# XJay18/NeuMA

Measured on AMD Instinct MI355X. Metric: sim+render frames/sec (fwd+bwd), 100k pts / 128^3 grid / 1080p, higher is better.
Workload: dtype f32; 1 GPU; metric: 100000 particles / 128^3 grid / 200000 Gaussians / 1920x1080; substeps_per_frame=20, views_per_frame=3, sh_degree=3, material=jelly_0300 + LoRA r16, parallelism=single GPU, start_state=rest

## Files before the change

### neuma_amd/csrc/nm_material.hip

```cpp
#include "nm_common.h"
#include "nm_grid.h"
#include <cstddef>

typedef float f4 __attribute__((ext_vector_type(4)));
#ifdef NM_PHASES
__device__ long long g_nm_phase[3 * 8 * 2048];
extern "C" int nm_debug_phases(long long* out, int n) {
  return hipMemcpyFromSymbol(out, HIP_SYMBOL(g_nm_phase), (size_t)n * sizeof(long long)) == hipSuccess ? 0 : -2;
}
#define NM_PH_DECL long long ph_t0 = clock64(); long long ph[8] = {0, 0, 0, 0, 0, 0, 0, 0};
#define NM_PH(i) { long long t1 = clock64(); ph[i] += t1 - ph_t0; ph_t0 = t1; }
#define NM_PH_STORE_K(kind) if ((threadIdx.x & 63) == 0) { int w = blockIdx.x * 4 + (threadIdx.x >> 6); if (w < 2048) for (int i = 0; i < 8; ++i) g_nm_phase[((kind) * 2048 + w) * 8 + i] = ph[i]; }
#define NM_PH_STORE NM_PH_STORE_K(0)
#else
#define NM_PH_STORE_K(kind)
#define NM_PH_DECL
#define NM_PH(i)
#define NM_PH_STORE
#endif
#define NM_MFMA(a, b, c) __builtin_amdgcn_mfma_f32_16x16x4f32((a), (b), (c), 0, 0, 0)
#define NM_SB_() __builtin_amdgcn_sched_barrier(0)

#define NM_BWD_GRID 256
#define NM_PRO_WGS 32
#define NM_PROLOGUE_SPLIT(pro) material_prologue(pro)
__device__ __forceinline__ bool material_prologue(const GridPrologue& pro) {
  if (pro.mode == 0) return false;
  const int mat = pro.mat_grid;
  if ((int)gridDim.x > mat) {
    if ((int)blockIdx.x < mat) return false;
    grid_prologue(pro, blockIdx.x - mat, gridDim.x - mat);
    return true;
  }
  grid_prologue(pro, blockIdx.x, gridDim.x);
  return false;
}
__device__ __forceinline__ bool material_prologue_fwd(const GridPrologue& pro) {
  if (pro.mode == 0) return false;
  const int mat = pro.mat_grid;
  if ((int)gridDim.x > mat) {
    if ((int)blockIdx.x < mat) return false;
    grid_prologue_clear(pro, blockIdx.x - mat, gridDim.x - mat);
    return true;
  }
  grid_prologue_clear(pro, blockIdx.x, gridDim.x);
  return false;
}
#define NM_W0 (64 * 13)
#define NM_W1 (64 * 64)
#define NM_W2 (9 * 64)
#define NM_WTOT (NM_W0 + NM_W1 + NM_W2)
#define NM_WACC_W0 (64 * 64)
#define NM_WACC_W2 (64 * 64 + 16 * 64)
#define NM_WACC (64 * 64 + 16 * 64 + 16 * 64)
__host__ __device__ inline int wacc_to_plain(int e) {
  const int reg = e & 3, lane = (e >> 2) & 63, blk = e >> 8, g = lane >> 4, j = lane & 15;
  if (blk < 16) return NM_W0 + (16 * (blk >> 2) + 4 * g + reg) * 64 + 16 * (blk & 3) + j;
  if (blk < 20) return j < 13 ? (16 * (blk - 16) + 4 * g + reg) * 13 + j : -1;
  return 4 * g + reg < 9 ? NM_W0 + NM_W1 + (4 * g + reg) * 64 + 16 * (blk - 20) + j : -1;
// ... 170 lines not shown
  __device__ __forceinline__ void operator()() const {}
};
template <int NFLOAT, class HOOK = NoHook>
__device__ __forceinline__ void stage_permuted(const float* __restrict__ wperm, float* dst, HOOK between = HOOK()) {
  constexpr int NV = NFLOAT / 4, PER = (NV + 255) / 256;
  float4 v[PER];
#pragma unroll
  for (int k = 0; k < PER; ++k) {
    int i = threadIdx.x + 256 * k;
    v[k] = i < NV ? reinterpret_cast<const float4*>(wperm)[i] : make_float4(0.f, 0.f, 0.f, 0.f);
  }
  NM_SB_();
  between();
  NM_SB_();
#pragma unroll
  for (int k = 0; k < PER; ++k) {
    int i = threadIdx.x + 256 * k;
    if (i < NV) reinterpret_cast<float4*>(dst)[i] = v[k];
  }
}
template <int NA, int NB, int NHOOK, class HOOK>
__device__ __forceinline__ void stage_permuted2(const float* __restrict__ srca, float* dsta, const float* __restrict__ srcb, float* dstb,
                                                HOOK between) {
  constexpr int VA = NA / 4, PA = (VA + 255) / 256, VB = NB / 4, PB = (VB + 255) / 256;
  f4 va[PA], vb[PB];
#pragma unroll
  for (int k = 0; k < PA; ++k) {
    const int i = threadIdx.x + 256 * k;
    const f4* ptr = reinterpret_cast<const f4*>(srca) + (i < VA ? i : VA - 1);
    asm volatile("global_load_dwordx4 %0, %1, off" : "=v"(va[k]) : "v"(ptr));
  }
#pragma unroll
  for (int k = 0; k < PB; ++k) {
    const int i = threadIdx.x + 256 * k;
    const f4* ptr = reinterpret_cast<const f4*>(srcb) + (i < VB ? i : VB - 1);
    asm volatile("global_load_dwordx4 %0, %1, off" : "=v"(vb[k]) : "v"(ptr));
  }
  asm volatile("" ::: "memory");
  between();
  static_assert(NHOOK >= 0 && NHOOK < 48, "vmcnt is a 6-bit counter");
  asm volatile("s_waitcnt vmcnt(%0)" ::"n"(NHOOK) : "memory");
#pragma unroll
  for (int k = 0; k < PA; ++k) {
    const int i = threadIdx.x + 256 * k;
    asm volatile("" : "+v"(va[k]));
    if (i < VA) *reinterpret_cast<f4*>(dsta + 4 * i) = va[k];
  }
#pragma unroll
  for (int k = 0; k < PB; ++k) {
    const int i = threadIdx.x + 256 * k;
    asm volatile("" : "+v"(vb[k]));
    if (i < VB) *reinterpret_cast<f4*>(dstb + 4 * i) = vb[k];
  }
}
__global__ void __launch_bounds__(256) k_permute_weights(const float* __restrict__ w0, const float* __restrict__ w1,
                                                         const float* __restrict__ w2, float* __restrict__ wperm,
                                                         const float* __restrict__ w0b, const float* __restrict__ w1b,
                                                         const float* __restrict__ w2b, float* __restrict__ wpermb) {
  __shared__ float raw[NM_RAWTOT];
  if (blockIdx.x == 1) { w0 = w0b; w1 = w1b; w2 = w2b; wperm = wpermb; }
  __shared__ float perm[NM_PERM_ALL];
  stage_raw_weights(w0, w1, w2, raw);
  __syncthreads();
  stage_fwd_weights(raw, perm, perm + 16 * 64, perm + 16 * 64 + 64 * 64);
  stage_bwd_weights(raw, perm + NM_PERM_FWD, perm + NM_PERM_FWD + 16 * 64, perm + NM_PERM_FWD + 16 * 64 + 64 * 64);
  __syncthreads();
  for (int i = threadIdx.x; i < NM_PERM_ALL; i += 256) wperm[i] = perm[i];
}

__device__ __forceinline__ void svd_store(float* __restrict__ dst, int n, int p, const M3& U, const float s[3], const M3& V) {
#pragma unroll
  for (int c = 0; c < 9; ++c) __builtin_nontemporal_store(U.m[c], &dst[(size_t)c * n + p]);
#pragma unroll
  for (int c = 0; c < 3; ++c) __builtin_nontemporal_store(s[c], &dst[(size_t)(9 + c) * n + p]);
#pragma unroll
  for (int c = 0; c < 9; ++c) __builtin_nontemporal_store(V.m[c], &dst[(size_t)(12 + c) * n + p]);
}
__device__ __forceinline__ void svd_load(const float* __restrict__ src, int n, int p, M3& U, float s[3], M3& V) {
#pragma unroll
  for (int c = 0; c < 9; ++c) U.m[c] = __builtin_nontemporal_load(&src[(size_t)c * n + p]);
#pragma unroll
  for (int c = 0; c < 3; ++c) s[c] = __builtin_nontemporal_load(&src[(size_t)(9 + c) * n + p]);
#pragma unroll
  for (int c = 0; c < 9; ++c) V.m[c] = __builtin_nontemporal_load(&src[(size_t)(12 + c) * n + p]);
}
template <bool HAVE_SVD = false>
__device__ __forceinline__ void nm_features(const M3& F, float z[13], M3& R, M3& U, M3& V, float s[3]) {
  if (!HAVE_SVD) nm_svd3(F, U, s, V);
  R = m3_mul_nt(U, V);
  M3 G = m3_mul_tn(F, F);
  z[0] = s[0] - 1.f; z[1] = s[1] - 1.f; z[2] = s[2] - 1.f;
#pragma unroll
  for (int i = 0; i < 9; ++i) z[3 + i] = G.m[i] - ((i % 4 == 0) ? 1.f : 0.f);
  z[12] = m3_det(F) - 1.f;
}

#define NM_SB() __builtin_amdgcn_sched_barrier(0)
template <int G>
struct AGroup {
  float a[G];
};
template <int G>
__device__ __forceinline__ void a_fetch(AGroup<G>& o, const float* __restrict__ base, int lane, int grp) {
  static_assert(G % 4 == 0, "groups of four operands (one 16-byte read each)");
#pragma unroll
  for (int q = 0; q < G / 4; ++q) {
// ... 303 lines not shown
    NM_LAUNCH(k_material_fwd_pair<true>, dim3(launch), dim3(256), 0, s, n, q, alpha_p, wperm_p, wperm_e, F_next, stress_next, gp, *g2p,
              svd_p, svd_e, ap, ae);
  else
    NM_LAUNCH(k_material_fwd_pair<false>, dim3(launch), dim3(256), 0, s, n, q, alpha_p, wperm_p, wperm_e, F_next, stress_next, gp, *g2p,
              svd_p, svd_e, ap, ae);
  NM_LAUNCH_CHECK();
  return NM_OK;
}
int nm_material_prepare(const nm_mlp* w, float* wperm, void* stream) {
  NM_LAUNCH(k_permute_weights, dim3(1), dim3(256), 0, (hipStream_t)stream, w->w0, w->w1, w->w2, wperm, (const float*)nullptr,
            (const float*)nullptr, (const float*)nullptr, (float*)nullptr);
  NM_LAUNCH_CHECK();
  return NM_OK;
}
int nm_material_prepare2(const nm_mlp* wa, float* wperm_a, const nm_mlp* wb, float* wperm_b, void* stream) {
  NM_LAUNCH(k_permute_weights, dim3(2), dim3(256), 0, (hipStream_t)stream, wa->w0, wa->w1, wa->w2, wperm_a, wb->w0, wb->w1, wb->w2,
            wperm_b);
  NM_LAUNCH_CHECK();
  return NM_OK;
}
size_t nm_material_prepared_floats() { return NM_PERM_ALL; }

extern "C" int nm_material_fwd(int32_t n, int32_t kind, float alpha, const float* F, const nm_mlp* w, float* out,
                               void* stream) {
  NM_REQUIRE(n >= 0, "negative n");
  NM_REQUIRE(kind == NM_ELASTICITY || kind == NM_PLASTICITY, "kind must be NM_ELASTICITY or NM_PLASTICITY");
  if (n == 0) return NM_OK;
  NM_REQUIRE(F && out && w && w->w0 && w->w1 && w->w2, "null pointer");
  return nm_material_fwd_launch(n, kind, alpha, F, w, nullptr, out, nullptr, nullptr, stream);
}

struct BwdFuse {
  const float* trial_C;
  const int* enabled;
  float dt;
  int add_to_gF;
  int polar;
  const float* svd_in;
};
struct BwdWave {
  float Z[64 * 17];
  float GY[64 * 13];
  float Y[64 * 9];
  float GZ[64 * 13];
  float TA[64 * 17];
  float TB[64 * 17];
  float TC[64 * 17];
};
struct BwdLds {
  float P0[16 * 64], P1[64 * 64], P2[16 * 64];
  float Q0[16 * 64], Q1[64 * 64], Q2[12 * 64];
  BwdWave W[4];
};

struct BwdArgs {
  int n, q;
  float alpha;
  const float *F, *w0, *w1, *w2, *wperm, *gout;
  float *gF, *wpart;
  int want_w;
  BwdFuse fz;
  const f4* act;
};

template <int KIND, bool ACT, bool WW = false>
__device__ __forceinline__ void material_bwd_body(const BwdArgs& a, char* smem_raw) {
  const int n = a.n, q = a.q, wmode = a.want_w;
  const bool want_w = WW ? true : (wmode != 0);
  const float alpha = a.alpha;
  const float* __restrict__ F = a.F;
  const float *__restrict__ w0 = a.w0, *__restrict__ w1 = a.w1, *__restrict__ w2 = a.w2, *__restrict__ wperm = a.wperm;
  const float* __restrict__ gout = a.gout;
  float *__restrict__ gF = a.gF, *__restrict__ wpart = a.wpart;
  const BwdFuse fz = a.fz;
  BwdLds& L = *reinterpret_cast<BwdLds*>(smem_raw);
  NM_PH_DECL
  const int wave = threadIdx.x >> 6, lane = threadIdx.x & 63;
  const int pbeg = min(n, (blockIdx.x * 4 + wave) * q), pend = min(n, pbeg + q);
  struct M3Raw {
    f4 a, b;
    float c;
  };
  typedef float f4u __attribute__((ext_vector_type(4), aligned(4)));
  auto raw_load = [](const float* __restrict__ ptr, M3Raw& r) {
    r.a = *reinterpret_cast<const f4u*>(ptr); r.b = *reinterpret_cast<const f4u*>(ptr + 4); r.c = ptr[8];
  };
  auto raw_m3 = [](const M3Raw& r) {
    M3 m;
    m.m[0] = r.a[0]; m.m[1] = r.a[1]; m.m[2] = r.a[2]; m.m[3] = r.a[3];
    m.m[4] = r.b[0]; m.m[5] = r.b[1]; m.m[6] = r.b[2]; m.m[7] = r.b[3]; m.m[8] = r.c;
    return m;
  };
  struct RoundIn {
    int en_p;
    M3Raw Fp, go, T;
    M3 U, V;
    float s[3];
  };
  f4 nx[ACT ? NM_ACT_SLOTS : 1];
  auto load_first_act = [&](int c0_) {
    if (ACT) {
      const f4* at_ = a.act + (size_t)(c0_ >> 4) * NM_ACT_SLOTS * 64 + lane;
#pragma unroll
      for (int k = 0; k < NM_ACT_SLOTS; ++k) nx[k] = __builtin_nontemporal_load(&at_[k * 64]);
    }
  };
  auto load_round = [&](int c0_, RoundIn& o) {
    const int p_ = c0_ + lane;
    const bool valid_ = p_ < pend;
    o.en_p = (fz.trial_C && valid_) ? fz.enabled[p_] : 0;
    if (valid_) {
      raw_load(F + (size_t)9 * p_, o.Fp);
      raw_load(gout + (size_t)9 * p_, o.go);
      if (fz.trial_C) raw_load(fz.trial_C + (size_t)9 * p_, o.T);
    }
    if (fz.svd_in) {
      if (valid_) svd_load(fz.svd_in, n, p_, o.U, o.s, o.V);
      else { o.U = m3_ident(); o.V = m3_ident(); o.s[0] = o.s[1] = o.s[2] = 1.f; }
    }
  };
  RoundIn ahead;
  if (pbeg < pend) load_round(pbeg, ahead);
  NM_SB();
  if (wperm) {
    static_assert(offsetof(BwdLds, W) == NM_PERM_ALL * sizeof(float), "P0..Q2 must be contiguous in operand order");
    if (ACT) {
      stage_permuted2<16 * 64, NM_PERM_ALL - NM_PERM_FWD, NM_ACT_SLOTS>(wperm, L.P0, wperm + NM_PERM_FWD, L.Q0,
                                                          [&]() { load_first_act(pbeg < pend ? pbeg : 0); });
    } else {
      stage_permuted<NM_PERM_ALL>(wperm, L.P0);
    }
    __syncthreads();
  } else {
    static_assert(sizeof(BwdWave) * 4 >= NM_RAWTOT * sizeof(float), "raw weights must fit the per-wave buffers");
    float* raw = &L.W[0].Z[0];
    stage_raw_weights(w0, w1, w2, raw);
    __syncthreads();
    stage_fwd_weights(raw, L.P0, L.P1, L.P2);
    stage_bwd_weights(raw, L.Q0, L.Q1, L.Q2);
    __syncthreads();
  }
  NM_PH(0)
  const int j = lane & 15, g = lane >> 4;
  float* zb = L.W[wave].Z;
  float* gyb = L.W[wave].GY;
  float* yb = L.W[wave].Y;
  float* gzb = L.W[wave].GZ;
  float* ta = L.W[wave].TA;
  float* tb = L.W[wave].TB;
  float* tc = L.W[wave].TC;
  const f4 zero = {0.f, 0.f, 0.f, 0.f};
  f4 gW1[4][4], gW0[4], gW2[4];
#pragma unroll
  for (int a = 0; a < 4; ++a) {
    gW0[a] = zero; gW2[a] = zero;
#pragma unroll
    for (int b = 0; b < 4; ++b) gW1[a][b] = zero;
  }
  for (int c0 = pbeg; c0 < pend; c0 += 64) {
    const int p = c0 + lane;
    const bool valid = p < pend;
    const int ntile = (min(64, pend - c0) + 15) >> 4;
    const f4* act_tile = ACT ? a.act + (size_t)(c0 >> 4) * NM_ACT_SLOTS * 64 + lane : nullptr;
    M3 Fp = valid ? raw_m3(ahead.Fp) : m3_ident(), go = valid ? raw_m3(ahead.go) : m3_zero();
    M3 T = (fz.trial_C && valid) ? raw_m3(ahead.T) : m3_zero();
    M3 R, U = ahead.U, V = ahead.V;
    float z[13], s[3] = {ahead.s[0], ahead.s[1], ahead.s[2]};
    const bool trial = ahead.en_p != 0;
    if (c0 + 64 < pend) load_round(c0 + 64, ahead);
    NM_SB();
    if (fz.trial_C && !trial) { Fp = m3_ident(); T = m3_zero(); }
    if (trial) {
#pragma unroll
      for (int i = 0; i < 9; ++i) T.m[i] *= fz.dt;
      T.m[0] += 1.f; T.m[4] += 1.f; T.m[8] += 1.f;
      Fp = m3_mul(T, Fp);
    }
    if (fz.svd_in) nm_features<true>(Fp, z, R, U, V, s);
    else nm_features(Fp, z, R, U, V, s);
#pragma unroll
    for (int c = 0; c < 13; ++c) zb[lane * 17 + c] = z[c];
    zb[lane * 17 + 13] = 0.f; zb[lane * 17 + 14] = 0.f; zb[lane * 17 + 15] = 0.f;
    M3 Rtg = m3_mul_tn(R, go);
    M3 Xb;
    if (KIND == NM_ELASTICITY) Xb = m3_mul(Rtg, Fp);
    else {
#pragma unroll
      for (int i = 0; i < 9; ++i) Xb.m[i] = alpha * Rtg.m[i];
    }
#pragma unroll
    for (int r = 0; r < 3; ++r)
#pragma unroll
      for (int c = 0; c < 3; ++c) gyb[lane * 13 + 3 * r + c] = 0.5f * (Xb.m[3 * r + c] + Xb.m[3 * c + r]);
    gyb[lane * 13 + 9] = 0.f; gyb[lane * 13 + 10] = 0.f; gyb[lane * 13 + 11] = 0.f; gyb[lane * 13 + 12] = 0.f;
    __builtin_amdgcn_wave_barrier();
    NM_PH(1)

#pragma unroll 1
    for (int ct = 0; ct < ntile; ++ct) {
      MlpFwd m;
      if (ACT) {
        f4 h2[4];
#pragma unroll
        for (int rt = 0; rt < 4; ++rt) { h2[rt] = nx[rt]; m.g2[rt] = nx[4 + rt]; }
        m.y = nx[8];
        const bool more = c0 + 16 * (ct + 1) < pend;
        if (more) {
#pragma unroll
          for (int k = 0; k < 5; ++k) nx[k] = __builtin_nontemporal_load(&act_tile[((size_t)(ct + 1) * NM_ACT_SLOTS + k) * 64]);
        }
        float zin[4];
#pragma unroll
        for (int ks = 0; ks < 4; ++ks) zin[ks] = zb[(ct * 16 + j) * 17 + 4 * ks + g];
        AGroup<8> first;
        a_fetch<8>(first, L.P0, lane, 0);
        const f4 zero4 = {0.f, 0.f, 0.f, 0.f};
        f4 a1[4] = {zero4, zero4, zero4, zero4};
        a_chain<16, 8, 3, 2>(first, L.P0, lane, zin, a1, [&]() {
          if (want_w) {
#pragma unroll
            for (int rt = 0; rt < 4; ++rt)
#pragma unroll
              for (int r = 0; r < 4; ++r) tb[(16 * rt + 4 * g + r) * 17 + j] = h2[rt][r];
            __builtin_amdgcn_wave_barrier();
          }
        });
#pragma unroll
        for (int rt = 0; rt < 4; ++rt)
#pragma unroll
          for (int pr = 0; pr < 2; ++pr) {
            f2 h, dh;
            nm_gelu_both2((f2){a1[rt][2 * pr], a1[rt][2 * pr + 1]}, h, dh);
            m.g1[rt][2 * pr] = dh[0];
            m.g1[rt][2 * pr + 1] = dh[1];
            if (want_w) {
              tc[(16 * rt + 4 * g + 2 * pr) * 17 + j] = h[0];
              tc[(16 * rt + 4 * g + 2 * pr + 1) * 17 + j] = h[1];
            }
          }
        __builtin_amdgcn_wave_barrier();
      } else {
        float zin[4];
#pragma unroll
        for (int ks = 0; ks < 4; ++ks) zin[ks] = zb[(ct * 16 + j) * 17 + 4 * ks + g];
        AGroup<8> first;
        a_fetch<8>(first, L.P0, lane, 0);
        mlp_forward_tile<true>(L.P0, L.P1, L.P2, zin, lane, first, m, want_w ? tc : nullptr, want_w ? tb : nullptr);
      }
#pragma unroll
      for (int r = 0; r < 4; ++r) {
        int row = 4 * g + r;
        if (row < 9) yb[(ct * 16 + j) * 9 + row] = m.y[r];
      }
      NM_PH(2)
      const float* gyt = gyb + ct * 16 * 13;
      f4 d2[4] = {zero, zero, zero, zero};
      float w2a[2], w2b[2][4];
      {
        AGroup<4> q2g;
        a_fetch<4>(q2g, L.Q2, lane, 0);
        float b[3];
#pragma unroll
        for (int ks = 0; ks < 3; ++ks) b[ks] = gyt[j * 13 + 4 * ks + g];
        if (want_w) {
          w2a[0] = j < 9 ? gyt[g * 13 + j] : 0.f;
#pragma unroll
          for (int ctp = 0; ctp < 4; ++ctp) w2b[0][ctp] = tb[(16 * ctp + j) * 17 + g];
        }
        a_chain<12, 4, 3, 2>(q2g, L.Q2, lane, b, d2);
      }
#pragma unroll
      for (int rt = 0; rt < 4; ++rt) d2[rt] *= m.g2[rt];
      NM_PH(4)
      AGroup<8> q1g;
      a_fetch<8>(q1g, L.Q1, lane, 0);
      NM_SB();
      if (want_w) {
#pragma unroll
        for (int rt = 0; rt < 4; ++rt)
#pragma unroll
          for (int r = 0; r < 4; ++r) ta[(16 * rt + 4 * g + r) * 17 + j] = d2[rt][r];
        __builtin_amdgcn_wave_barrier();
#pragma unroll
        for (int ks = 0; ks < 4; ++ks) {
          const int c = ks & 1, nx = c ^ 1;
          if (ks < 3) {
            w2a[nx] = j < 9 ? gyt[(4 * (ks + 1) + g) * 13 + j] : 0.f;
#pragma unroll
            for (int ctp = 0; ctp < 4; ++ctp) w2b[nx][ctp] = tb[(16 * ctp + j) * 17 + 4 * (ks + 1) + g];
          }
          NM_SB();
#pragma unroll
          for (int ctp = 0; ctp < 4; ++ctp) gW2[ctp] = NM_MFMA(w2a[c], w2b[c][ctp], gW2[ctp]);
          NM_SB();
        }
      }
      NM_PH(3)
      if (ACT && c0 + 16 * (ct + 1) < pend) {
#pragma unroll
        for (int k = 5; k < NM_ACT_SLOTS; ++k) nx[k] = __builtin_nontemporal_load(&act_tile[((size_t)(ct + 1) * NM_ACT_SLOTS + k) * 64]);
      }
      f4 d1[4] = {zero, zero, zero, zero};
      float w1a[2][4], w1b[2][4];
      {
        float b[16];
#pragma unroll
        for (int rtp = 0; rtp < 4; ++rtp)
#pragma unroll
          for (int reg = 0; reg < 4; ++reg) b[4 * rtp + reg] = d2[rtp][reg];
        if (want_w) {
#pragma unroll
          for (int t = 0; t < 4; ++t) {
            w1b[0][t] = tc[(16 * t + j) * 17 + g];
            w1a[0][t] = ta[(16 * t + j) * 17 + g];
          }
        }
        a_chain<64, 8, 3, 2>(q1g, L.Q1, lane, b, d1);
      }
#pragma unroll
      for (int rt = 0; rt < 4; ++rt) d1[rt] *= m.g1[rt];
      NM_PH(6)
      AGroup<8> q0g;
      a_fetch<8>(q0g, L.Q0, lane, 0);
      NM_SB();
      if (want_w) {
#pragma unroll
        for (int rt = 0; rt < 4; ++rt)
#pragma unroll
          for (int r = 0; r < 4; ++r) tb[(16 * rt + 4 * g + r) * 17 + j] = d1[rt][r];
        __builtin_amdgcn_wave_barrier();
#pragma unroll
        for (int ks = 0; ks < 4; ++ks) {
          const int c = ks & 1, nx = c ^ 1;
          if (ks < 3) {
#pragma unroll
            for (int t = 0; t < 4; ++t) {
              w1b[nx][t] = tc[(16 * t + j) * 17 + 4 * (ks + 1) + g];
              w1a[nx][t] = ta[(16 * t + j) * 17 + 4 * (ks + 1) + g];
            }
          }
          NM_SB();
#pragma unroll
          for (int rt = 0; rt < 4; ++rt)
#pragma unroll
            for (int ctp = 0; ctp < 4; ++ctp) gW1[rt][ctp] = NM_MFMA(w1a[c][rt], w1b[c][ctp], gW1[rt][ctp]);
          NM_SB();
        }
      }
      NM_PH(5)
      f4 dzz[2] = {zero, zero};
      float w0b[2], w0a[2][4];
      {
        float b[16];
#pragma unroll
        for (int rtp = 0; rtp < 4; ++rtp)
#pragma unroll
          for (int reg = 0; reg < 4; ++reg) b[4 * rtp + reg] = d1[rtp][reg];
        if (want_w) {
          w0b[0] = zb[(ct * 16 + g) * 17 + j];
#pragma unroll
          for (int rt = 0; rt < 4; ++rt) w0a[0][rt] = tb[(16 * rt + j) * 17 + g];
        }
        a_chain<16, 8, 1, 0>(q0g, L.Q0, lane, b, dzz);
      }
      const f4 dza = dzz[0] + dzz[1];
#pragma unroll
      for (int r = 0; r < 4; ++r) {
        int row = 4 * g + r;
        if (row < 13) gzb[(ct * 16 + j) * 13 + row] = dza[r];
      }
      if (want_w) {
#pragma unroll
        for (int ks = 0; ks < 4; ++ks) {
          const int c = ks & 1, nx = c ^ 1;
          if (ks < 3) {
            w0b[nx] = zb[(ct * 16 + 4 * (ks + 1) + g) * 17 + j];
#pragma unroll
            for (int rt = 0; rt < 4; ++rt) w0a[nx][rt] = tb[(16 * rt + j) * 17 + 4 * (ks + 1) + g];
          }
          NM_SB();
#pragma unroll
          for (int rt = 0; rt < 4; ++rt) gW0[rt] = NM_MFMA(w0a[c][rt], w0b[c], gW0[rt]);
          NM_SB();
        }
      }
    }
    __builtin_amdgcn_wave_barrier();

    M3Raw prev_raw;
    const bool add_prev = fz.add_to_gF && valid;
    if (add_prev) raw_load(gF + (size_t)9 * p, prev_raw);
    M3 X;
#pragma unroll
    for (int i = 0; i < 9; ++i) X.m[i] = yb[lane * 9 + i];
    M3 Xs;
#pragma unroll
    for (int r = 0; r < 3; ++r)
#pragma unroll
      for (int c = 0; c < 3; ++c) Xs.m[3 * r + c] = 0.5f * (X.m[3 * r + c] + X.m[3 * c + r]);
    float zbv[13];
#pragma unroll
    for (int c = 0; c < 13; ++c) zbv[c] = gzb[lane * 13 + c];
    M3 Fb, Rb;
    if (KIND == NM_ELASTICITY) {
      M3 gFm = m3_mul(go, Fp);
      Rb = m3_mul(gFm, Xs);
      M3 RX = m3_mul(R, Xs);
      Fb = m3_mul_tn(go, RX);
    } else {
      M3 gX = m3_mul(go, Xs);
#pragma unroll
      for (int i = 0; i < 9; ++i) { Rb.m[i] = alpha * gX.m[i]; Fb.m[i] = go.m[i]; }
    }
    M3 At = m3_mul(m3_mul_tn(U, Rb), V);
    M3 inner;
#pragma unroll
    for (int r = 0; r < 3; ++r)
#pragma unroll
      for (int c = 0; c < 3; ++c) {
        if (r == c) { inner.m[4 * r] = zbv[r]; continue; }
        float kf;
        if (fz.polar) {
          float den = s[r] + s[c];
          den = fabsf(den) < 1e-6f ? copysignf(1e-6f, den) : den;
          kf = 1.f / den;
        } else {
          const int a = r < c ? r : c, b = r < c ? c : r;
          kf = (s[b] - s[a]) / fminf(s[b] * s[b] - s[a] * s[a], -1e-6f);
        }
        inner.m[3 * r + c] = (At.m[3 * r + c] - At.m[3 * c + r]) * kf;
      }
    M3 t = m3_mul_nt(m3_mul(U, inner), V);
    M3 Gs;
#pragma unroll
    for (int r = 0; r < 3; ++r)
#pragma unroll
      for (int c = 0; c < 3; ++c) Gs.m[3 * r + c] = zbv[3 + 3 * r + c] + zbv[3 + 3 * c + r];
    M3 FG = m3_mul(Fp, Gs);
    M3 cof = m3_cofactor(Fp);
#pragma unroll
    for (int i = 0; i < 9; ++i) Fb.m[i] += t.m[i] + FG.m[i] + zbv[12] * cof.m[i];
    if (valid) {
      if (add_prev) {
        const M3 prev = raw_m3(prev_raw);
#pragma unroll
        for (int i = 0; i < 9; ++i) Fb.m[i] += prev.m[i];
      }
      m3_store(gF + 9 * p, Fb);
    }
    __builtin_amdgcn_wave_barrier();
    NM_PH(7)
  }
  NM_PH_STORE_K(KIND == NM_PLASTICITY ? 1 : 0)

  if (!want_w) return;
  constexpr int W4 = NM_WACC / 4, WPER = W4 / 256;
  static_assert(W4 % 256 == 0, "whole 16-byte pieces per thread");
  f4* dst = reinterpret_cast<f4*>(wpart + (size_t)blockIdx.x * NM_WACC);
  f4 prev[WPER];
  if (wmode == 2) {
#pragma unroll
    for (int k = 0; k < WPER; ++k) prev[k] = dst[threadIdx.x + 256 * k];
  } else {
#pragma unroll
    for (int k = 0; k < WPER; ++k) prev[k] = zero;
  }
  NM_SB();
  __syncthreads();
  static_assert(sizeof(BwdLds) >= 4 * NM_WACC * sizeof(float), "four weight-gradient copies must fit");
  f4* red = reinterpret_cast<f4*>(smem_raw) + wave * W4;
#pragma unroll
  for (int rt = 0; rt < 4; ++rt) {
#pragma unroll
    for (int ctp = 0; ctp < 4; ++ctp) red[(rt * 4 + ctp) * 64 + lane] = gW1[rt][ctp];
    red[NM_WACC_W0 / 4 + rt * 64 + lane] = gW0[rt];
    red[NM_WACC_W2 / 4 + rt * 64 + lane] = gW2[rt];
  }
  __syncthreads();
  const f4* all = reinterpret_cast<const f4*>(smem_raw);
#pragma unroll
  for (int k = 0; k < WPER; ++k) {
    const int i = threadIdx.x + 256 * k;
    const f4 v = (all[i] + all[W4 + i]) + (all[2 * W4 + i] + all[3 * W4 + i]);
    dst[i] = prev[k] + v;
  }
}

template <int KIND, bool ACT>
__global__ void __launch_bounds__(256, 1) k_material_bwd(BwdArgs a, GridPrologue pro) {
  extern __shared__ __attribute__((aligned(16))) char smem_raw[];
  if (NM_PROLOGUE_SPLIT(pro)) return;
  material_bwd_body<KIND, ACT>(a, smem_raw);
}

template <bool ACT, bool WW>
__global__ void __launch_bounds__(256, 1) k_material_bwd_pair(BwdArgs e, BwdArgs p, GridPrologue pro) {
  extern __shared__ __attribute__((aligned(16))) char smem_raw[];
  if (NM_PROLOGUE_SPLIT(pro)) return;
  material_bwd_body<NM_ELASTICITY, ACT, WW>(e, smem_raw);
  __threadfence_block();
  __syncthreads();
  material_bwd_body<NM_PLASTICITY, ACT, WW>(p, smem_raw);
}

__global__ void __launch_bounds__(256) k_wgrad_reduce(const float* __restrict__ wpart, int nparts, float* __restrict__ g0,
                                                      float* __restrict__ g1, float* __restrict__ g2, int accumulate,
                                                      const float* __restrict__ wpart_b, float* __restrict__ gb) {
  __shared__ float part[4][64];
  if (blockIdx.y == 1) {
    wpart = wpart_b; g0 = gb; g1 = gb + NM_W0; g2 = gb + NM_W0 + NM_W1;
  }
  const int li = threadIdx.x & 63, sl = threadIdx.x >> 6;
  const int e = blockIdx.x * 64 + li;
  const int i = wacc_to_plain(e);
  float acc = 0.f;
  if (i >= 0) {
    float a0 = 0.f, a1 = 0.f, a2 = 0.f, a3 = 0.f;
    int b = sl;
    for (; b + 12 < nparts; b += 16) {
      a0 += wpart[(size_t)b * NM_WACC + e];
      a1 += wpart[(size_t)(b + 4) * NM_WACC + e];
      a2 += wpart[(size_t)(b + 8) * NM_WACC + e];
      a3 += wpart[(size_t)(b + 12) * NM_WACC + e];
    }
    for (; b < nparts; b += 4) a0 += wpart[(size_t)b * NM_WACC + e];
    acc = (a0 + a1) + (a2 + a3);
  }
  part[sl][li] = acc;
  __syncthreads();
  if (sl == 0 && i >= 0) {
    acc = (part[0][li] + part[1][li]) + (part[2][li] + part[3][li]);
    float* dst = i < NM_W0 ? g0 + i : (i < NM_W0 + NM_W1 ? g1 + (i - NM_W0) : g2 + (i - NM_W0 - NM_W1));
    *dst = accumulate ? *dst + acc : acc;
  }
}

static int bwd_attr_once() {
  static bool attr_done[64] = {};
  int devid = 0;
  NM_HIP_CHECK(hipGetDevice(&devid));
  const bool attr_set = devid >= 0 && devid < 64 && attr_done[devid];
  if (!attr_set) {
    NM_HIP_CHECK(hipFuncSetAttribute((const void*)k_material_bwd<NM_ELASTICITY, true>, hipFuncAttributeMaxDynamicSharedMemorySize,
                                     (int)sizeof(BwdLds)));
    NM_HIP_CHECK(hipFuncSetAttribute((const void*)k_material_bwd<NM_PLASTICITY, true>, hipFuncAttributeMaxDynamicSharedMemorySize,
                                     (int)sizeof(BwdLds)));
    NM_HIP_CHECK(hipFuncSetAttribute((const void*)k_material_bwd_pair<true, true>, hipFuncAttributeMaxDynamicSharedMemorySize,
                                     (int)sizeof(BwdLds)));
    NM_HIP_CHECK(hipFuncSetAttribute((const void*)k_material_bwd_pair<true, false>, hipFuncAttributeMaxDynamicSharedMemorySize,
                                     (int)sizeof(BwdLds)));
    NM_HIP_CHECK(hipFuncSetAttribute((const void*)k_material_bwd<NM_ELASTICITY, false>, hipFuncAttributeMaxDynamicSharedMemorySize,
                                     (int)sizeof(BwdLds)));
    NM_HIP_CHECK(hipFuncSetAttribute((const void*)k_material_bwd<NM_PLASTICITY, false>, hipFuncAttributeMaxDynamicSharedMemorySize,
                                     (int)sizeof(BwdLds)));
    NM_HIP_CHECK(hipFuncSetAttribute((const void*)k_material_bwd_pair<false, true>, hipFuncAttributeMaxDynamicSharedMemorySize,
                                     (int)sizeof(BwdLds)));
    NM_HIP_CHECK(hipFuncSetAttribute((const void*)k_material_bwd_pair<false, false>, hipFuncAttributeMaxDynamicSharedMemorySize,
                                     (int)sizeof(BwdLds)));
    if (devid >= 0 && devid < 64) attr_done[devid] = true;
  }
  return NM_OK;
}
static BwdArgs bwd_args(int32_t n, int q, float alpha, const float* F, const nm_mlp* w, const float* wperm, const float* gout,
                        float* gF, float* wpart, int wmode, const float* trial_C, const int* enabled, float dt, int flags,
                        const float* svd_in = nullptr, const float* act = nullptr) {
  BwdArgs a;
  a.n = n; a.q = q; a.alpha = alpha; a.F = F;
  a.w0 = w ? w->w0 : nullptr; a.w1 = w ? w->w1 : nullptr; a.w2 = w ? w->w2 : nullptr;
  a.wperm = wperm; a.gout = gout; a.gF = gF; a.wpart = wpart; a.want_w = wmode;
  a.fz.trial_C = trial_C; a.fz.enabled = enabled; a.fz.dt = dt; a.fz.add_to_gF = flags & 1; a.fz.polar = (flags >> 1) & 1;
  a.fz.svd_in = svd_in;
  a.act = reinterpret_cast<const f4*>(act);
  return a;
}

int nm_material_bwd_launch(int32_t n, int32_t kind, float alpha, const float* F, const nm_mlp* w, const float* wperm,
                           const float* gout, float* gF, float* wpart, int wmode, const float* trial_C, const int* enabled,
                           float dt, int add_to_gF, const GridPrologue* pro, void* stream, const float* svd_in, const float* act) {
  GridPrologue gp;
  if (pro) gp = *pro; else { memset(&gp, 0, sizeof(gp)); }
  hipStream_t s = (hipStream_t)stream;
  int grid, q;
  nm_wave_quota(n, grid, q);
  gp.mat_grid = grid;
  const int launch = (pro && grid + NM_PRO_WGS <= NM_BWD_GRID) ? grid + NM_PRO_WGS : grid;
  int rc = bwd_attr_once();
  if (rc) return rc;
  BwdArgs a = bwd_args(n, q, alpha, F, w, wperm, gout, gF, wpart, wmode, trial_C, enabled, dt, add_to_gF, svd_in, act);
  if (kind == NM_ELASTICITY && act)
    NM_LAUNCH((k_material_bwd<NM_ELASTICITY, true>), dim3(launch), dim3(256), sizeof(BwdLds), s, a, gp);
  else if (kind == NM_ELASTICITY)
    NM_LAUNCH((k_material_bwd<NM_ELASTICITY, false>), dim3(launch), dim3(256), sizeof(BwdLds), s, a, gp);
  else if (act)
    NM_LAUNCH((k_material_bwd<NM_PLASTICITY, true>), dim3(launch), dim3(256), sizeof(BwdLds), s, a, gp);
  else
    NM_LAUNCH((k_material_bwd<NM_PLASTICITY, false>), dim3(launch), dim3(256), sizeof(BwdLds), s, a, gp);
  NM_LAUNCH_CHECK();
  return NM_OK;
}

int nm_material_bwd_pair_launch(int32_t n, const float* F_e, const nm_mlp* we, const float* wperm_e, const float* gS, float* gF,
                                float* wpart_e, int wmode_e, float alpha_p, const float* F_p, const nm_mlp* wp,
                                const float* wperm_p, float* gFtrial, float* wpart_p, int wmode_p, const float* trial_C,
                                const int* enabled, float dt, int polar, const GridPrologue* pro, void* stream,
                                const float* svd_in_e, const float* svd_in_p, const float* act_e, const float* act_p) {
  GridPrologue gp;
  if (pro) gp = *pro; else { memset(&gp, 0, sizeof(gp)); }
  hipStream_t s = (hipStream_t)stream;
  int grid, q;
  nm_wave_quota(n, grid, q);
  gp.mat_grid = grid;
  const int launch = (pro && grid + NM_PRO_WGS <= NM_BWD_GRID) ? grid + NM_PRO_WGS : grid;
  int rc = bwd_attr_once();
  if (rc) return rc;
  BwdArgs e = bwd_args(n, q, 0.f, F_e, we, wperm_e, gS, gF, wpart_e, wmode_e, nullptr, nullptr, 0.f, 1 | (polar ? 2 : 0), svd_in_e, act_e);
  BwdArgs p = bwd_args(n, q, alpha_p, F_p, wp, wperm_p, gF, gFtrial, wpart_p, wmode_p, trial_C, enabled, dt, polar ? 2 : 0, svd_in_p, act_p);
  const bool ww = wmode_e != 0 && wmode_p != 0;
  if (act_e && act_p && ww)
    NM_LAUNCH((k_material_bwd_pair<true, true>), dim3(launch), dim3(256), sizeof(BwdLds), s, e, p, gp);
  else if (act_e && act_p)
    NM_LAUNCH((k_material_bwd_pair<true, false>), dim3(launch), dim3(256), sizeof(BwdLds), s, e, p, gp);
  else if (ww)
    NM_LAUNCH((k_material_bwd_pair<false, true>), dim3(launch), dim3(256), sizeof(BwdLds), s, e, p, gp);
  else
    NM_LAUNCH((k_material_bwd_pair<false, false>), dim3(launch), dim3(256), sizeof(BwdLds), s, e, p, gp);
  NM_LAUNCH_CHECK();
  return NM_OK;
}
int nm_material_wgrad_reduce(const float* wpart, int32_t n, float* gw0, float* gw1, float* gw2, int accumulate, void* stream) {
  int grid, q;
  nm_wave_quota(n, grid, q);
  NM_LAUNCH(k_wgrad_reduce, dim3(NM_WACC / 64), dim3(256), 0, (hipStream_t)stream, wpart, grid, gw0, gw1, gw2,
                     accumulate, (const float*)nullptr, (float*)nullptr);
  NM_LAUNCH_CHECK();
  return NM_OK;
}
int nm_material_wgrad_reduce2(const float* wpart_a, const float* wpart_b, int32_t n, float* gw_a, float* gw_b, void* stream) {
  int grid, q;
  nm_wave_quota(n, grid, q);
  NM_LAUNCH(k_wgrad_reduce, dim3(NM_WACC / 64, 2), dim3(256), 0, (hipStream_t)stream, wpart_a, grid, gw_a, gw_a + NM_W0,
            gw_a + NM_W0 + NM_W1, 0, wpart_b, gw_b);
  NM_LAUNCH_CHECK();
  return NM_OK;
}

extern "C" size_t nm_material_bwd_workspace(int32_t n) {
  (void)n;
  return (size_t)NM_BWD_GRID * NM_WACC * sizeof(float);
}

extern "C" int nm_material_bwd(int32_t n, int32_t kind, float alpha, const float* F, const nm_mlp* w, const float* gout,
                               float* gF, float* gw0, float* gw1, float* gw2, void* workspace, size_t workspace_bytes,
                               void* stream) {
  return nm_material_bwd_ex(n, kind, alpha, F, w, gout, gF, gw0, gw1, gw2, 0, workspace, workspace_bytes, stream);
}

extern "C" int nm_material_bwd_ex(int32_t n, int32_t kind, float alpha, const float* F, const nm_mlp* w, const float* gout,
                                  float* gF, float* gw0, float* gw1, float* gw2, int32_t flags, void* workspace,
                                  size_t workspace_bytes, void* stream) {
  const int accumulate = flags & NM_BWD_ACCUMULATE;
  NM_REQUIRE(n >= 0, "negative n");
  NM_REQUIRE(kind == NM_ELASTICITY || kind == NM_PLASTICITY, "kind must be NM_ELASTICITY or NM_PLASTICITY");
  const int want_w = (gw0 && gw1 && gw2) ? 1 : 0;
  NM_REQUIRE(want_w || (!gw0 && !gw1 && !gw2), "weight gradient outputs must be all set or all NULL");
  hipStream_t s = (hipStream_t)stream;
  if (n == 0) {
    if (want_w && !accumulate) {
      NM_HIP_CHECK(hipMemsetAsync(gw0, 0, NM_W0 * sizeof(float), s));
      NM_HIP_CHECK(hipMemsetAsync(gw1, 0, NM_W1 * sizeof(float), s));
      NM_HIP_CHECK(hipMemsetAsync(gw2, 0, NM_W2 * sizeof(float), s));
    }
// ... 159 lines not shown
```

Before: 199.8 frames/s.

## Keep both nets' backward operands resident in LDS and prefetch second net early

Adds a resident LDS layout for the paired elastic/plastic backward kernel. Both networks' permuted operand blocks are staged into LDS once at kernel start, so the second net needs no second weight staging. The first net's last round also prefetches the second net's particle data and activation cache, so the second body starts without a cold load. In exchange LDS use grows, and the cross-net prefetch path adds complexity, such as an explicit vmcnt(0) wait and pointer switching.

```diff
diff --git a/neuma_amd/csrc/nm_material.hip b/neuma_amd/csrc/nm_material.hip
--- a/neuma_amd/csrc/nm_material.hip
+++ b/neuma_amd/csrc/nm_material.hip
@@ -4,7 +4,7 @@
 
 typedef float f4 __attribute__((ext_vector_type(4)));
 #ifdef NM_PHASES
-__device__ long long g_nm_phase[3 * 8 * 2048];
+__device__ long long g_nm_phase[4 * 8 * 2048];
 extern "C" int nm_debug_phases(long long* out, int n) {
   return hipMemcpyFromSymbol(out, HIP_SYMBOL(g_nm_phase), (size_t)n * sizeof(long long)) == hipSuccess ? 0 : -2;
 }
@@ -281,6 +281,49 @@
     asm volatile("" : "+v"(vb[k]));
     if (i < VB) *reinterpret_cast<f4*>(dstb + 4 * i) = vb[k];
   }
+}
+template <int NFLOAT>
+struct StageRegs {
+  f4 v[(NFLOAT / 4 + 255) / 256];
+};
+template <int NFLOAT>
+__device__ __forceinline__ void stage_issue(const float* __restrict__ src, StageRegs<NFLOAT>& r) {
+  constexpr int NV = NFLOAT / 4, PER = (NV + 255) / 256;
+#pragma unroll
+  for (int k = 0; k < PER; ++k) {
+    const int i = threadIdx.x + 256 * k;
+    const f4* ptr = reinterpret_cast<const f4*>(src) + (i < NV ? i : NV - 1);
+    asm volatile("global_load_dwordx4 %0, %1, off" : "=v"(r.v[k]) : "v"(ptr));
+  }
+}
+template <int NFLOAT>
+__device__ __forceinline__ void stage_write(float* dst, StageRegs<NFLOAT>& r) {
+  constexpr int NV = NFLOAT / 4, PER = (NV + 255) / 256;
+#pragma unroll
+  for (int k = 0; k < PER; ++k) {
+    const int i = threadIdx.x + 256 * k;
+    asm volatile("" : "+v"(r.v[k]));
+    if (i < NV) *reinterpret_cast<f4*>(dst + 4 * i) = r.v[k];
+  }
+}
+template <int NA, int NB, int NHOOK, class HOOK>
+__device__ __forceinline__ void stage_permuted4(const float* __restrict__ a0, float* da0, const float* __restrict__ b0, float* db0,
+                                                const float* __restrict__ a1, float* da1, const float* __restrict__ b1, float* db1,
+                                                HOOK between) {
+  StageRegs<NA> ra0, ra1;
+  StageRegs<NB> rb0, rb1;
+  stage_issue(a0, ra0);
+  stage_issue(b0, rb0);
+  stage_issue(a1, ra1);
+  stage_issue(b1, rb1);
+  asm volatile("" ::: "memory");
+  between();
+  static_assert(NHOOK >= 0 && NHOOK < 48, "vmcnt is a 6-bit counter");
+  asm volatile("s_waitcnt vmcnt(%0)" ::"n"(NHOOK) : "memory");
+  stage_write(da0, ra0);
+  stage_write(db0, rb0);
+  stage_write(da1, ra1);
+  stage_write(db1, rb1);
 }
 __global__ void __launch_bounds__(256) k_permute_weights(const float* __restrict__ w0, const float* __restrict__ w1,
                                                          const float* __restrict__ w2, float* __restrict__ wperm,
@@ -690,6 +733,17 @@
   float Q0[16 * 64], Q1[64 * 64], Q2[12 * 64];
   BwdWave W[4];
 };
+struct BwdNetOps {
+  float P0[16 * 64];
+  float Q0[16 * 64], Q1[64 * 64], Q2[12 * 64];
+};
+struct BwdLdsPair {
+  BwdNetOps N[2];
+  BwdWave W[4];
+};
+static_assert(sizeof(BwdLdsPair) <= 160 * 1024, "both nets' operands and the per-wave buffers must fit one CU's LDS");
+static_assert(offsetof(BwdNetOps, Q0) == 16 * 64 * sizeof(float) && sizeof(BwdNetOps) == (16 * 64 + NM_PERM_ALL - NM_PERM_FWD) * sizeof(float),
+              "P0 | Q0 | Q1 | Q2 contiguous");
 
 struct BwdArgs {
   int n, q;
@@ -700,9 +754,24 @@
   BwdFuse fz;
   const f4* act;
 };
-
-template <int KIND, bool ACT, bool WW = false>
-__device__ __forceinline__ void material_bwd_body(const BwdArgs& a, char* smem_raw) {
+struct M3Raw {
+  f4 a, b;
+  float c;
+};
+struct RoundIn {
+  int en_p;
+  M3Raw Fp, go, T;
+  M3 U, V;
+  float s[3];
+};
+struct BwdCarry {
+  RoundIn ahead;
+  f4 nx[NM_ACT_SLOTS];
+};
+
+template <int KIND, bool ACT, bool WW = false, int RES = 0>
+__device__ __forceinline__ void material_bwd_body(const BwdArgs& a, char* smem_raw, BwdCarry& cr, const BwdArgs& nb) {
+  static_assert(RES == 0 || ACT, "the resident layout holds the activation-cache operands only");
   const int n = a.n, q = a.q, wmode = a.want_w;
   const bool want_w = WW ? true : (wmode != 0);
   const float alpha = a.alpha;
@@ -712,13 +781,15 @@
   float *__restrict__ gF = a.gF, *__restrict__ wpart = a.wpart;
   const BwdFuse fz = a.fz;
   BwdLds& L = *reinterpret_cast<BwdLds*>(smem_raw);
+  BwdLdsPair& LP = *reinterpret_cast<BwdLdsPair*>(smem_raw);
+  BwdNetOps& LN = LP.N[RES == 2 ? 1 : 0];
+  const float *sP0 = RES ? LN.P0 : L.P0, *sP1 = RES ? nullptr : L.P1, *sP2 = RES ? nullptr : L.P2;
+  const float *sQ0 = RES ? LN.Q0 : L.Q0, *sQ1 = RES ? LN.Q1 : L.Q1, *sQ2 = RES ? LN.Q2 : L.Q2;
+  BwdWave* const Wv = RES ? LP.W : L.W;
   NM_PH_DECL
   const int wave = threadIdx.x >> 6, lane = threadIdx.x & 63;
   const int pbeg = min(n, (blockIdx.x * 4 + wave) * q), pend = min(n, pbeg + q);
-  struct M3Raw {
-    f4 a, b;
-    float c;
-  };
+  const bool early = RES != 0 && pend - pbeg > 64;
   typedef float f4u __attribute__((ext_vector_type(4), aligned(4)));
   auto raw_load = [](const float* __restrict__ ptr, M3Raw& r) {
     r.a = *reinterpret_cast<const f4u*>(ptr); r.b = *reinterpret_cast<const f4u*>(ptr + 4); r.c = ptr[8];
@@ -729,13 +800,7 @@
     m.m[4] = r.b[0]; m.m[5] = r.b[1]; m.m[6] = r.b[2]; m.m[7] = r.b[3]; m.m[8] = r.c;
     return m;
   };
-  struct RoundIn {
-    int en_p;
-    M3Raw Fp, go, T;
-    M3 U, V;
-    float s[3];
-  };
-  f4 nx[ACT ? NM_ACT_SLOTS : 1];
+  f4(&nx)[NM_ACT_SLOTS] = cr.nx;
   auto load_first_act = [&](int c0_) {
     if (ACT) {
       const f4* at_ = a.act + (size_t)(c0_ >> 4) * NM_ACT_SLOTS * 64 + lane;
@@ -743,50 +808,65 @@
       for (int k = 0; k < NM_ACT_SLOTS; ++k) nx[k] = __builtin_nontemporal_load(&at_[k * 64]);
     }
   };
-  auto load_round = [&](int c0_, RoundIn& o) {
+  auto load_round_of = [&](const float* __restrict__ F_, const float* __restrict__ gout_, const BwdFuse& fz_, int c0_, RoundIn& o) {
     const int p_ = c0_ + lane;
     const bool valid_ = p_ < pend;
-    o.en_p = (fz.trial_C && valid_) ? fz.enabled[p_] : 0;
+    o.en_p = (fz_.trial_C && valid_) ? fz_.enabled[p_] : 0;
     if (valid_) {
-      raw_load(F + (size_t)9 * p_, o.Fp);
-      raw_load(gout + (size_t)9 * p_, o.go);
-      if (fz.trial_C) raw_load(fz.trial_C + (size_t)9 * p_, o.T);
-    }
-    if (fz.svd_in) {
-      if (valid_) svd_load(fz.svd_in, n, p_, o.U, o.s, o.V);
+      raw_load(F_ + (size_t)9 * p_, o.Fp);
+      raw_load(gout_ + (size_t)9 * p_, o.go);
+      if (fz_.trial_C) raw_load(fz_.trial_C + (size_t)9 * p_, o.T);
+    }
+    if (fz_.svd_in) {
+      if (valid_) svd_load(fz_.svd_in, n, p_, o.U, o.s, o.V);
       else { o.U = m3_ident(); o.V = m3_ident(); o.s[0] = o.s[1] = o.s[2] = 1.f; }
     }
   };
-  RoundIn ahead;
-  if (pbeg < pend) load_round(pbeg, ahead);
-  NM_SB();
-  if (wperm) {
-    static_assert(offsetof(BwdLds, W) == NM_PERM_ALL * sizeof(float), "P0..Q2 must be contiguous in operand order");
-    if (ACT) {
-      stage_permuted2<16 * 64, NM_PERM_ALL - NM_PERM_FWD, NM_ACT_SLOTS>(wperm, L.P0, wperm + NM_PERM_FWD, L.Q0,
-                                                          [&]() { load_first_act(pbeg < pend ? pbeg : 0); });
+  auto load_round = [&](int c0_, RoundIn& o) { load_round_of(F, gout, fz, c0_, o); };
+  RoundIn& ahead = cr.ahead;
+  if (RES == 2) {
+    if (!early && pbeg < pend) {
+      load_round(pbeg, ahead);
+      load_first_act(pbeg);
+    }
+    NM_SB();
+  } else {
+    if (pbeg < pend) load_round(pbeg, ahead);
+    NM_SB();
+    if (RES == 1) {
+      constexpr int NQ = NM_PERM_ALL - NM_PERM_FWD;
+      stage_permuted4<16 * 64, NQ, NM_ACT_SLOTS>(wperm, LP.N[0].P0, wperm + NM_PERM_FWD, LP.N[0].Q0, nb.wperm, LP.N[1].P0,
+                                                 nb.wperm + NM_PERM_FWD, LP.N[1].Q0,
+                                                 [&]() { load_first_act(pbeg < pend ? pbeg : 0); });
+      __syncthreads();
+    } else if (wperm) {
+      static_assert(offsetof(BwdLds, W) == NM_PERM_ALL * sizeof(float), "P0..Q2 must be contiguous in operand order");
+      if (ACT) {
+        stage_permuted2<16 * 64, NM_PERM_ALL - NM_PERM_FWD, NM_ACT_SLOTS>(wperm, L.P0, wperm + NM_PERM_FWD, L.Q0,
+                                                            [&]() { load_first_act(pbeg < pend ? pbeg : 0); });
+      } else {
+        stage_permuted<NM_PERM_ALL>(wperm, L.P0);
+      }
+      __syncthreads();
     } else {
-      stage_permuted<NM_PERM_ALL>(wperm, L.P0);
-    }
-    __syncthreads();
-  } else {
-    static_assert(sizeof(BwdWave) * 4 >= NM_RAWTOT * sizeof(float), "raw weights must fit the per-wave buffers");
-    float* raw = &L.W[0].Z[0];
-    stage_raw_weights(w0, w1, w2, raw);
-    __syncthreads();
-    stage_fwd_weights(raw, L.P0, L.P1, L.P2);
-    stage_bwd_weights(raw, L.Q0, L.Q1, L.Q2);
-    __syncthreads();
+      static_assert(sizeof(BwdWave) * 4 >= NM_RAWTOT * sizeof(float), "raw weights must fit the per-wave buffers");
+      float* raw = &L.W[0].Z[0];
+      stage_raw_weights(w0, w1, w2, raw);
+      __syncthreads();
+      stage_fwd_weights(raw, L.P0, L.P1, L.P2);
+      stage_bwd_weights(raw, L.Q0, L.Q1, L.Q2);
+      __syncthreads();
+    }
   }
   NM_PH(0)
   const int j = lane & 15, g = lane >> 4;
-  float* zb = L.W[wave].Z;
-  float* gyb = L.W[wave].GY;
-  float* yb = L.W[wave].Y;
-  float* gzb = L.W[wave].GZ;
-  float* ta = L.W[wave].TA;
-  float* tb = L.W[wave].TB;
-  float* tc = L.W[wave].TC;
+  float* zb = Wv[wave].Z;
+  float* gyb = Wv[wave].GY;
+  float* yb = Wv[wave].Y;
+  float* gzb = Wv[wave].GZ;
+  float* ta = Wv[wave].TA;
+  float* tb = Wv[wave].TB;
+  float* tc = Wv[wave].TC;
   const f4 zero = {0.f, 0.f, 0.f, 0.f};
   f4 gW1[4][4], gW0[4], gW2[4];
 #pragma unroll
@@ -805,7 +885,12 @@
     M3 R, U = ahead.U, V = ahead.V;
     float z[13], s[3] = {ahead.s[0], ahead.s[1], ahead.s[2]};
     const bool trial = ahead.en_p != 0;
-    if (c0 + 64 < pend) load_round(c0 + 64, ahead);
+    if (RES == 1) {
+      const bool more_rounds = c0 + 64 < pend, first2 = early && !more_rounds;
+      if (first2) asm volatile("s_waitcnt vmcnt(0)" ::: "memory");
+      if (more_rounds || first2)
+        load_round_of(first2 ? nb.F : F, first2 ? nb.gout : gout, first2 ? nb.fz : fz, first2 ? pbeg : c0 + 64, ahead);
+    } else if (c0 + 64 < pend) load_round(c0 + 64, ahead);
     NM_SB();
     if (fz.trial_C && !trial) { Fp = m3_ident(); T = m3_zero(); }
     if (trial) {
@@ -843,18 +928,21 @@
         for (int rt = 0; rt < 4; ++rt) { h2[rt] = nx[rt]; m.g2[rt] = nx[4 + rt]; }
         m.y = nx[8];
         const bool more = c0 + 16 * (ct + 1) < pend;
-        if (more) {
-#pragma unroll
-          for (int k = 0; k < 5; ++k) nx[k] = __builtin_nontemporal_load(&act_tile[((size_t)(ct + 1) * NM_ACT_SLOTS + k) * 64]);
+        const bool warm = RES == 1 && early && !more;
+        const f4* act_next = &act_tile[(size_t)(ct + 1) * NM_ACT_SLOTS * 64];
+        if (RES == 1 && warm) act_next = nb.act + (size_t)(pbeg >> 4) * NM_ACT_SLOTS * 64 + lane;
+        if (more || warm) {
+#pragma unroll
+          for (int k = 0; k < 5; ++k) nx[k] = __builtin_nontemporal_load(&act_next[(size_t)k * 64]);
         }
         float zin[4];
 #pragma unroll
         for (int ks = 0; ks < 4; ++ks) zin[ks] = zb[(ct * 16 + j) * 17 + 4 * ks + g];
         AGroup<8> first;
-        a_fetch<8>(first, L.P0, lane, 0);
+        a_fetch<8>(first, sP0, lane, 0);
         const f4 zero4 = {0.f, 0.f, 0.f, 0.f};
         f4 a1[4] = {zero4, zero4, zero4, zero4};
-        a_chain<16, 8, 3, 2>(first, L.P0, lane, zin, a1, [&]() {
+        a_chain<16, 8, 3, 2>(first, sP0, lane, zin, a1, [&]() {
           if (want_w) {
 #pragma unroll
             for (int rt = 0; rt < 4; ++rt)
@@ -882,8 +970,8 @@
 #pragma unroll
         for (int ks = 0; ks < 4; ++ks) zin[ks] = zb[(ct * 16 + j) * 17 + 4 * ks + g];
         AGroup<8> first;
-        a_fetch<8>(first, L.P0, lane, 0);
-        mlp_forward_tile<true>(L.P0, L.P1, L.P2, zin, lane, first, m, want_w ? tc : nullptr, want_w ? tb : nullptr);
+        a_fetch<8>(first, sP0, lane, 0);
+        mlp_forward_tile<true>(sP0, sP1, sP2, zin, lane, first, m, want_w ? tc : nullptr, want_w ? tb : nullptr);
       }
 #pragma unroll
       for (int r = 0; r < 4; ++r) {
@@ -896,7 +984,7 @@
       float w2a[2], w2b[2][4];
       {
         AGroup<4> q2g;
-        a_fetch<4>(q2g, L.Q2, lane, 0);
+        a_fetch<4>(q2g, sQ2, lane, 0);
         float b[3];
 #pragma unroll
         for (int ks = 0; ks < 3; ++ks) b[ks] = gyt[j * 13 + 4 * ks + g];
@@ -905,13 +993,13 @@
 #pragma unroll
           for (int ctp = 0; ctp < 4; ++ctp) w2b[0][ctp] = tb[(16 * ctp + j) * 17 + g];
         }
-        a_chain<12, 4, 3, 2>(q2g, L.Q2, lane, b, d2);
+        a_chain<12, 4, 3, 2>(q2g, sQ2, lane, b, d2);
       }
 #pragma unroll
       for (int rt = 0; rt < 4; ++rt) d2[rt] *= m.g2[rt];
       NM_PH(4)
       AGroup<8> q1g;
-      a_fetch<8>(q1g, L.Q1, lane, 0);
+      a_fetch<8>(q1g, sQ1, lane, 0);
       NM_SB();
       if (want_w) {
 #pragma unroll
@@ -934,9 +1022,14 @@
         }
       }
       NM_PH(3)
-      if (ACT && c0 + 16 * (ct + 1) < pend) {
-#pragma unroll
-        for (int k = 5; k < NM_ACT_SLOTS; ++k) nx[k] = __builtin_nontemporal_load(&act_tile[((size_t)(ct + 1) * NM_ACT_SLOTS + k) * 64]);
+      if (ACT) {
+        const bool more = c0 + 16 * (ct + 1) < pend, warm = RES == 1 && early && !more;
+        const f4* act_next = &act_tile[(size_t)(ct + 1) * NM_ACT_SLOTS * 64];
+        if (RES == 1 && warm) act_next = nb.act + (size_t)(pbeg >> 4) * NM_ACT_SLOTS * 64 + lane;
+        if (more || warm) {
+#pragma unroll
+          for (int k = 5; k < NM_ACT_SLOTS; ++k) nx[k] = __builtin_nontemporal_load(&act_next[(size_t)k * 64]);
+        }
       }
       f4 d1[4] = {zero, zero, zero, zero};
       float w1a[2][4], w1b[2][4];
@@ -953,13 +1046,13 @@
             w1a[0][t] = ta[(16 * t + j) * 17 + g];
           }
         }
-        a_chain<64, 8, 3, 2>(q1g, L.Q1, lane, b, d1);
+        a_chain<64, 8, 3, 2>(q1g, sQ1, lane, b, d1);
       }
 #pragma unroll
       for (int rt = 0; rt < 4; ++rt) d1[rt] *= m.g1[rt];
       NM_PH(6)
       AGroup<8> q0g;
-      a_fetch<8>(q0g, L.Q0, lane, 0);
+      a_fetch<8>(q0g, sQ0, lane, 0);
       NM_SB();
       if (want_w) {
 #pragma unroll
@@ -999,7 +1092,7 @@
 #pragma unroll
           for (int rt = 0; rt < 4; ++rt) w0a[0][rt] = tb[(16 * rt + j) * 17 + g];
         }
-        a_chain<16, 8, 1, 0>(q0g, L.Q0, lane, b, dzz);
+        a_chain<16, 8, 1, 0>(q0g, sQ0, lane, b, dzz);
       }
       const f4 dza = dzz[0] + dzz[1];
 #pragma unroll
@@ -1089,7 +1182,7 @@
     __builtin_amdgcn_wave_barrier();
     NM_PH(7)
   }
-  NM_PH_STORE_K(KIND == NM_PLASTICITY ? 1 : 0)
+  NM_PH_STORE_K(RES == 1 ? 3 : KIND == NM_PLASTICITY ? 1 : 0)
 
   if (!want_w) return;
   constexpr int W4 = NM_WACC / 4, WPER = W4 / 256;
@@ -1106,7 +1199,9 @@
   NM_SB();
   __syncthreads();
   static_assert(sizeof(BwdLds) >= 4 * NM_WACC * sizeof(float), "four weight-gradient copies must fit");
-  f4* red = reinterpret_cast<f4*>(smem_raw) + wave * W4;
+  static_assert(sizeof(BwdWave) * 4 >= 4 * NM_WACC * sizeof(float), "four weight-gradient copies must fit the per-wave buffers");
+  char* const red_raw = RES ? reinterpret_cast<char*>(LP.W) : smem_raw;
+  f4* red = reinterpret_cast<f4*>(red_raw) + wave * W4;
 #pragma unroll
   for (int rt = 0; rt < 4; ++rt) {
 #pragma unroll
@@ -1115,7 +1210,7 @@
     red[NM_WACC_W2 / 4 + rt * 64 + lane] = gW2[rt];
   }
   __syncthreads();
-  const f4* all = reinterpret_cast<const f4*>(smem_raw);
+  const f4* all = reinterpret_cast<const f4*>(red_raw);
 #pragma unroll
   for (int k = 0; k < WPER; ++k) {
     const int i = threadIdx.x + 256 * k;
@@ -1128,17 +1223,19 @@
 __global__ void __launch_bounds__(256, 1) k_material_bwd(BwdArgs a, GridPrologue pro) {
   extern __shared__ __attribute__((aligned(16))) char smem_raw[];
   if (NM_PROLOGUE_SPLIT(pro)) return;
-  material_bwd_body<KIND, ACT>(a, smem_raw);
-}
-
-template <bool ACT, bool WW>
+  BwdCarry cr;
+  material_bwd_body<KIND, ACT>(a, smem_raw, cr, a);
+}
+
+template <bool ACT, bool WW, bool RES = false>
 __global__ void __launch_bounds__(256, 1) k_material_bwd_pair(BwdArgs e, BwdArgs p, GridPrologue pro) {
   extern __shared__ __attribute__((aligned(16))) char smem_raw[];
   if (NM_PROLOGUE_SPLIT(pro)) return;
-  material_bwd_body<NM_ELASTICITY, ACT, WW>(e, smem_raw);
+  BwdCarry cr;
+  material_bwd_body<NM_ELASTICITY, ACT, WW, RES ? 1 : 0>(e, smem_raw, cr, p);
   __threadfence_block();
   __syncthreads();
-  material_bwd_body<NM_PLASTICITY, ACT, WW>(p, smem_raw);
+  material_bwd_body<NM_PLASTICITY, ACT, WW, RES ? 2 : 0>(p, smem_raw, cr, p);
 }
 
 __global__ void __launch_bounds__(256) k_wgrad_reduce(const float* __restrict__ wpart, int nparts, float* __restrict__ g0,
@@ -1187,6 +1284,10 @@
                                      (int)sizeof(BwdLds)));
     NM_HIP_CHECK(hipFuncSetAttribute((const void*)k_material_bwd_pair<true, false>, hipFuncAttributeMaxDynamicSharedMemorySize,
                                      (int)sizeof(BwdLds)));
+    NM_HIP_CHECK(hipFuncSetAttribute((const void*)k_material_bwd_pair<true, true, true>, hipFuncAttributeMaxDynamicSharedMemorySize,
+                                     (int)sizeof(BwdLdsPair)));
+    NM_HIP_CHECK(hipFuncSetAttribute((const void*)k_material_bwd_pair<true, false, true>, hipFuncAttributeMaxDynamicSharedMemorySize,
+                                     (int)sizeof(BwdLdsPair)));
     NM_HIP_CHECK(hipFuncSetAttribute((const void*)k_material_bwd<NM_ELASTICITY, false>, hipFuncAttributeMaxDynamicSharedMemorySize,
                                      (int)sizeof(BwdLds)));
     NM_HIP_CHECK(hipFuncSetAttribute((const void*)k_material_bwd<NM_PLASTICITY, false>, hipFuncAttributeMaxDynamicSharedMemorySize,
@@ -1254,7 +1355,12 @@
   BwdArgs e = bwd_args(n, q, 0.f, F_e, we, wperm_e, gS, gF, wpart_e, wmode_e, nullptr, nullptr, 0.f, 1 | (polar ? 2 : 0), svd_in_e, act_e);
   BwdArgs p = bwd_args(n, q, alpha_p, F_p, wp, wperm_p, gF, gFtrial, wpart_p, wmode_p, trial_C, enabled, dt, polar ? 2 : 0, svd_in_p, act_p);
   const bool ww = wmode_e != 0 && wmode_p != 0;
-  if (act_e && act_p && ww)
+  const bool resident = act_e && act_p && wperm_e && wperm_p;
+  if (resident && ww)
+    NM_LAUNCH((k_material_bwd_pair<true, true, true>), dim3(launch), dim3(256), sizeof(BwdLdsPair), s, e, p, gp);
+  else if (resident)
+    NM_LAUNCH((k_material_bwd_pair<true, false, true>), dim3(launch), dim3(256), sizeof(BwdLdsPair), s, e, p, gp);
+  else if (act_e && act_p && ww)
     NM_LAUNCH((k_material_bwd_pair<true, true>), dim3(launch), dim3(256), sizeof(BwdLds), s, e, p, gp);
   else if (act_e && act_p)
     NM_LAUNCH((k_material_bwd_pair<true, false>), dim3(launch), dim3(256), sizeof(BwdLds), s, e, p, gp);
```

Result: no change. 201.3 frames/s (median of 6 runs) (+0.7%).
